# alebal123bal/BayesOpt_smart

Measured on AMD Instinct MI355X. Metric: candidate-points/sec (GP predict + HVI) at N_train=512, N_cand=1M, higher is better.
Workload: dtype f64; 1 GPU; C3: 2D/2-obj toy_function, N_train=512, N_cand=1,048,576 per GPU ('ij' integer grid), HVI (Sigma-UCB), q=3; n_train=512, n_cand_per_gpu=1048576, n_cand_total=1048576, n_objectives=2, dim=2, topq=3, parallelism=candidate-shard x1, step_launch=hip_graph, candidate_offset=0

## Files before the change

### bayesopt_smart_amd/csrc/bo_gridconv.hip

```cpp

#include "bo_predict_impl.h"

namespace {

using namespace bo;

constexpr int kListWaves = 4;
constexpr int kListChunk = 512;
#ifndef BO_ACC_RB
#define BO_ACC_RB 8
#endif
constexpr int kAccRB = BO_ACC_RB;
constexpr int kAccRows = 64 * kAccRB;
constexpr int kAccUnroll = 4;
constexpr int kClassLists = kConvClasses * kConvShards;
static_assert(kClassLists % 64 == 0 && kClassLists <= 2 * 64 * kConvAccWaves &&
              (kConvShards & (kConvShards - 1)) == 0 && kConvShards <= 16 && kConvShards <= kConvCountStride,
              "conv_acc_kernel's scan and lookup of the class lists");
#ifndef BO_CONV_PF
#define BO_CONV_PF 3
#endif
constexpr int kConvPF = BO_CONV_PF;
constexpr int kContractWaves = 8;
constexpr size_t kConvLdsBytes = 160 * 1024;
constexpr double kPairDrop = 0x1p-100;
constexpr double kTabFlush = 0x1p-128;

struct ListLds {
  int order, rc, nm;
  size_t bytes;
  __host__ __device__ ListLds(int n, int C)
      : order(C + 1), rc(order + n), nm(rc + 2 * n), bytes((size_t)(nm + kListWaves * kListChunk) * sizeof(int)) {}
};
struct AccLds {
  int ints, part;
  size_t bytes;
  __host__ __device__ explicit AccLds(int R)
      : ints(4 * R), part(kClassLists + 1),
        bytes((size_t)ints * sizeof(double) + (size_t)(part + kConvAccWaves + 1) / 2 * 2 * sizeof(int)) {}
};
struct ContractLds {
  int HB, tabH, hband, cn;
  size_t bytes;
  __host__ __device__ ContractLds(int C, int Cpad, int LT, int NP, int lists = 0)
      : HB(Cpad + LT / 2), tabH(2 * HB), hband(tabH + Cpad + C - 1), cn(hband + 1),
        bytes((size_t)cn * sizeof(double) + (size_t)NP * sizeof(int)) {
    if (bytes < (size_t)lists * sizeof(TopEntry)) bytes = (size_t)lists * sizeof(TopEntry);
  }
};

__device__ __forceinline__ void conv_list_done(const ConvArgs& a, int tau, int kept, int lane, int dyn) {
  if (kept == 0) {
    for (int o = 0; o < a.n_obj; ++o) {
      double* row = a.T + ((size_t)o * a.LT + tau) * a.ldr;
      for (int i = lane; i < a.ldr; i += 64) row[i] = 0.0;
    }
  }
  if (lane == 0) {
    a.pkept[tau] = kept;
    if (dyn && kept > 0) {
      const int e = 31 - __clz(kept);
      const int cls = 2 * e + (e > 0 ? (kept >> (e - 1)) & 1 : 0);
      const int sh = tau & (kConvShards - 1);
      const int slot = atomicAdd(a.ccount + cls * kConvCountStride + sh, 1);
      a.clist[(size_t)(cls * kConvShards + sh) * (a.LT / kConvShards) + slot] = tau;
    }
  }
}

__global__ __launch_bounds__(64 * kListWaves) void conv_list_kernel(const ConvArgs a, int tau_blocks, int dyn) {
  if (__builtin_amdgcn_readfirstlane(*a.flag) != 0) return;
  const int tid = threadIdx.x;
  if ((int)blockIdx.x >= tau_blocks) {
    const long long total = (long long)a.NP * a.ldr;
    const long long stride = (long long)(gridDim.x - tau_blocks) * (64 * kListWaves);
    for (int o = 0; o < a.n_obj; ++o) {
      const double nhl = a.nhl[o], pv = a.pv[o];
      double* tm = a.Tm + (size_t)o * a.NP * a.ldr;
      for (long long t = (long long)(blockIdx.x - tau_blocks) * (64 * kListWaves) + tid; t < total; t += stride) {
        const int s = (int)(t / a.ldr), i = (int)(t - (long long)s * a.ldr);
        double v = 0.0;
        if (s < a.n && i < a.nrows) {
          const int n = a.order[s];
          const double d = (double)(a.row_lo + i - a.rc[2 * n]);
          v = pv * a.alpha[(size_t)o * a.n_pad + n] * exp(nhl * (d * d));
        }
        tm[t] = v;
      }
    }
    return;
  }
  extern __shared__ __attribute__((aligned(16))) int si[];
  const ListLds L(a.n, a.C);
  int* cstart = si;
  int* order = si + L.order;
  int* rc = si + L.rc;
  for (int t = tid; t <= a.C; t += 64 * kListWaves) cstart[t] = a.cstart[t];
  for (int t = tid; t < a.n; t += 64 * kListWaves) order[t] = a.order[t];
  for (int t = tid; t < 2 * a.n; t += 64 * kListWaves) rc[t] = a.rc[t];
  __syncthreads();
  const int lane = tid & 63, wave = tid >> 6;
  int* nm = si + L.nm + wave * kListChunk;
  const int tau = blockIdx.x * kListWaves + wave;
  if (tau >= a.LT) return;
  int s0 = 0, s1 = 0;
  for (int c = lane; c < a.C; c += 64) {
    const int h = cstart[c + 1] - cstart[c];
    const int x0 = tau - c, x1 = x0 + 1;
    s0 += h * cstart[x0 < 0 ? 0 : x0 > a.C ? a.C : x0];
    s1 += h * cstart[x1 < 0 ? 0 : x1 > a.C ? a.C : x1];
  }
#pragma unroll
  for (int d = 32; d > 0; d >>= 1) {
    s0 += __shfl_xor(s0, d, 64);
    s1 += __shfl_xor(s1, d, 64);
  }
  const int h0 = (tau + 1) >> 1, h1 = (tau + 2) >> 1;
  const int p0 = __builtin_amdgcn_readfirstlane((s0 + cstart[h0 > a.C ? a.C : h0]) >> 1);
  const int total = __builtin_amdgcn_readfirstlane((s1 + cstart[h1 > a.C ? a.C : h1]) >> 1) - p0;
  if (lane == 0) a.pstart[tau] = p0;
  if (total == 0) {
    conv_list_done(a, tau, 0, lane, dyn);
    return;
  }
  const int R2 = 2 * a.R;
  const int per = (a.n + 63) / 64;
  const int n_lo = lane * per < a.n ? lane * per : a.n;
  const int n_hi = n_lo + per < a.n ? n_lo + per : a.n;
// ... 86 lines not shown
    const double* e = tb + s;
#pragma unroll
    for (int k = 0; k < kAccRB; ++k) ev[k] = e[it[k]];
  };
  auto term = [&](double wv, const double (&ev)[kAccRB]) {
#pragma unroll
    for (int k = 0; k < kAccRB; ++k) {
      const double t = __dmul_rn(wv, ev[k]);
      const double te = __builtin_fma(wv, ev[k], -t);
      const double s2 = __dadd_rn(hi[k], t);
      const double bb = __dsub_rn(s2, hi[k]);
      const double se = __dadd_rn(__dsub_rn(hi[k], __dsub_rn(s2, bb)), __dsub_rn(t, bb));
      hi[k] = s2;
      lo[k] = __dadd_rn(lo[k], __dadd_rn(se, te));
    }
  };
  int p = 0;
  for (; p + kAccUnroll <= cnt; p += kAccUnroll) {
    double wv[kAccUnroll];
    int sv[kAccUnroll];
#pragma unroll
    for (int u = 0; u < kAccUnroll; ++u) {
      wv[u] = w[p + u];
      sv[u] = sl[p + u];
    }
    double ev[2][kAccRB];
    gather(sv[0], ev[0]);
#pragma unroll
    for (int u = 0; u < kAccUnroll; ++u) {
      if (u + 1 < kAccUnroll) gather(sv[u + 1], ev[(u + 1) & 1]);
      term(wv[u], ev[u & 1]);
    }
  }
  for (; p < cnt; ++p) {
    double ev[kAccRB];
    gather(sl[p], ev);
    term(w[p], ev);
  }
#pragma unroll
  for (int k = 0; k < kAccRB; ++k) {
    const int i = ib + lane + 64 * k;
    if (FULL) Trow[i] = hi[k] + lo[k];
    else if (i < ldr) Trow[i] = i < nrows ? hi[k] + lo[k] : 0.0;
  }
}

__global__ __launch_bounds__(64 * kConvAccWaves) void conv_acc_kernel(
    const ConvArgs a, const double* __restrict__ pair_w, const int* __restrict__ pair_sl,
    const int* __restrict__ pstart, const int* __restrict__ pkept, const int* __restrict__ ccount,
    const int* __restrict__ clist, int* __restrict__ ticket, double* __restrict__ T, int nrb, int ngrp, int dyn) {
  if (__builtin_amdgcn_readfirstlane(*a.flag) != 0) return;
  extern __shared__ __attribute__((aligned(16))) double sd[];
  const int tid = threadIdx.x, lane = tid & 63, o = blockIdx.y;
  const double nhl = a.nhl[o];
  const int R2 = 2 * a.R;
  const AccLds L(a.R);
  double* tabE = sd;
  int* cst = (int*)(sd + L.ints);
  int* part = cst + L.part;
  for (int t = tid; t < 2 * R2; t += 64 * kConvAccWaves) {
    const int par = t >= R2 ? 1 : 0, h = t - par * R2;
    const double m = (double)(2 * h + par - (R2 - 2));
    tabE[t] = exp(0.5 * nhl * (m * m));
  }
  if (dyn) {
    int c[2], sum = 0;
#pragma unroll
    for (int u = 0; u < 2; ++u) {
      const int j = 2 * tid + u;
      c[u] = j < kClassLists ? ccount[(kConvClasses - 1 - j / kConvShards) * kConvCountStride + j % kConvShards] : 0;
      sum += c[u];
    }
    int incl = sum;
#pragma unroll
    for (int d = 1; d < 64; d <<= 1) {
      const int v = __shfl_up(incl, d, 64);
      if (lane >= d) incl += v;
    }
    if (lane == 63) part[tid >> 6] = incl;
    __syncthreads();
    int run = incl - sum;
    for (int w = 0; w < (tid >> 6); ++w) run += part[w];
#pragma unroll
    for (int u = 0; u < 2; ++u) {
      const int j = 2 * tid + u;
      if (j < kClassLists) cst[j] = run;
      run += c[u];
      if (j == kClassLists - 1) cst[kClassLists] = run;
    }
  }
  __syncthreads();
  const int n_items = (dyn ? cst[kClassLists] : a.LT) * nrb;
  const double* wo = pair_w + (size_t)o * a.n_pairs;
  const int g = blockIdx.x % ngrp;
  int* tk = ticket + (o * kConvTicketGroups + g) * kConvTicketStride;
  for (int k = (blockIdx.x / ngrp) * kConvAccWaves + (tid >> 6);;) {
    const int t = k * ngrp + g;
    if (t >= n_items) break;
    int nx = 0;
    if (dyn && lane == 0) nx = atomicAdd(tk, 1);
    const int oi = t / nrb, rb = t - oi * nrb;
    int tau = oi;
    if (dyn) {
      constexpr int per = kClassLists / 64;
      const unsigned long long b1 = __ballot(cst[per * lane + per] > oi);
      const int l1 = __builtin_ctzll(b1);
      const unsigned long long b2 = __ballot(cst[per * l1 + (lane < per ? lane : per - 1) + 1] > oi);
      const int j = per * l1 + __builtin_ctzll(b2);
      const int cls = kConvClasses - 1 - j / kConvShards;
      const int* list = clist + (size_t)(cls * kConvShards + j % kConvShards) * (a.LT / kConvShards);
      tau = __builtin_amdgcn_readfirstlane(list[oi - cst[j]]);
    }
    const int p0 = __builtin_amdgcn_readfirstlane(pstart[tau]);
    const int cnt = __builtin_amdgcn_readfirstlane(pkept[tau]);
    if (!dyn && cnt == 0) break;
    const int ib = rb * kAccRows;
    double* Trow = T + ((size_t)o * a.LT + tau) * a.ldr;
// ... 13 lines not shown
#pragma unroll
  for (int s = 0; s < 4; ++s) v[s] = p[(size_t)s * ldr];
#endif
}

template <int NB, class BGen>
__device__ __forceinline__ void conv_gemm(const double* __restrict__ X, int ldr, int nkb, int g, d4 (&acc)[NB],
                                          BGen&& bgen) {
  double ring[kConvPF][4];
#pragma unroll
  for (int p = 0; p < kConvPF; ++p) conv_load_a(X, ldr, p < nkb ? p : nkb - 1, g, ring[p]);
  for (int kb0 = 0; kb0 < nkb; kb0 += kConvPF) {
#pragma unroll
    for (int p = 0; p < kConvPF; ++p) {
      const int kb = kb0 + p;
      if (kb < nkb) {
        double av[4];
#pragma unroll
        for (int s = 0; s < 4; ++s) av[s] = ring[p][s];
        const int nx = kb + kConvPF;
        conv_load_a(X, ldr, nx < nkb ? nx : nkb - 1, g, ring[p]);
        double bv[4][NB];
        bgen(kb, bv);
#pragma unroll
        for (int s = 0; s < 4; ++s)
#pragma unroll
          for (int nb = 0; nb < NB; ++nb) acc[nb] = mfma64(av[s], bv[s][nb], acc[nb]);
      }
    }
  }
}

template <int NB>
__global__ __launch_bounds__(64 * kContractWaves) void conv_contract_kernel(const ConvArgs a) {
  if (__builtin_amdgcn_readfirstlane(*a.flag) != 0) return;
  extern __shared__ __attribute__((aligned(16))) double sd[];
  const ContractLds L(a.C, a.Cpad, a.LT, a.NP);
  double* tabB = sd;
  double* tabH = sd + L.tabH;
  int* hband = (int*)(sd + L.hband);
  int* cn = (int*)(sd + L.cn);
  constexpr int TW = 16 * NB;
  const int tid = threadIdx.x, lane = tid & 63, wave = tid >> 6;
  const int nt = blockDim.x, W = nt >> 6;
  const int g = lane >> 4, jl = lane & 15;
  const int cb_n = a.Cpad / TW;
  const long long n_wt = (long long)(a.ldr / 16) * cb_n;
  const long long gi_lo = a.cand_offset, gi_hi = a.cand_offset + a.n_cand;
#ifndef BO_ABL_CT_NOOUT
  const bool outs = true;
#else
  const bool outs = a.ld_out < 0;
#endif
  for (int t = tid; t < a.NP; t += nt) cn[t] = t < a.n ? a.rc[2 * a.order[t] + 1] : 0;

  double lv = -__builtin_inf();
  long long li = -1;
  double tab_nhl = __builtin_nan("");
  for (long long base = (long long)blockIdx.x * W; base < n_wt; base += (long long)gridDim.x * W) {
    const long long wt = base + wave;
    const bool active = wt < n_wt;
    const long long wtc = active ? wt : n_wt - 1;
    const int i0 = (int)(wtc / cb_n) * 16, j0 = (int)(wtc % cb_n) * TW;
    double acq[NB][4];
    for (int o = 0; o < a.n_obj; ++o) {
      const double nhl = a.nhl[o];
      if (!(nhl == tab_nhl)) {
        __syncthreads();
        int mq = 0;
        int mm = 0;
#ifndef BO_ABL_CT_NOTAB
        for (int t = tid; t < 2 * L.HB; t += nt) {
          const int par = t >= L.HB ? 1 : 0, h = t - par * L.HB;
          const int mi = 2 * h + par - (a.LT - 1);
          const double m = (double)mi;
          const double v = exp(0.5 * nhl * (m * m));
          const bool flush = v < kTabFlush;
          tabB[t] = flush ? 0.0 : v;
          if (!flush) mq = max(mq, abs(mi));
        }
        for (int t = tid; t < a.Cpad + a.C - 1; t += nt) {
          const int mi = t - (a.C - 1);
          const double m = (double)mi;
          const double v = exp(nhl * (m * m));
          const bool flush = v < kTabFlush;
          tabH[t] = flush ? 0.0 : v;
          if (!flush) mm = max(mm, abs(mi));
        }
#else
        mm = min((int)sqrt(128.0 * 0.6931471805599453 / -nhl), a.C - 1);
        mq = min((int)sqrt(256.0 * 0.6931471805599453 / -nhl), a.LT - 1);
#endif
        if (tid < 2) hband[tid] = 0;
        __syncthreads();
#pragma unroll
        for (int d = 32; d > 0; d >>= 1) {
          mq = max(mq, __shfl_xor(mq, d, 64));
          mm = max(mm, __shfl_xor(mm, d, 64));
        }
        if (lane == 0) {
          atomicMax(hband, mq);
          atomicMax(hband + 1, mm);
        }
        __syncthreads();
        tab_nhl = nhl;
      }
      int kq_lo = 0, kq_hi = a.LT / 16;
      if (!a.full) {
        const int hq = hband[0];
        const int t_hi = 2 * (j0 + TW - 1) + hq < a.LT - 1 ? 2 * (j0 + TW - 1) + hq : a.LT - 1;
        const int t_lo = 2 * j0 - hq > 0 ? (2 * j0 - hq < t_hi ? 2 * j0 - hq : t_hi) : 0;
        kq_lo = __builtin_amdgcn_readfirstlane(t_lo >> 4);
        kq_hi = __builtin_amdgcn_readfirstlane((t_hi >> 4) + 1);
      }
      d4 aq[NB], am[NB];
#pragma unroll
      for (int nb = 0; nb < NB; ++nb) {
        aq[nb] = (d4){0.0, 0.0, 0.0, 0.0};
        am[nb] = (d4){0.0, 0.0, 0.0, 0.0};
      }
      const double* Tq = a.T + ((size_t)o * a.LT + 16 * kq_lo) * a.ldr + i0 + jl;
      int km_lo = 0, km_hi = a.NP / 16;
      if (!a.full) {
        const int hm = hband[1];
        const int c_hi = j0 + TW + hm < a.C ? j0 + TW + hm : a.C;
        const int c_lo = j0 - hm > 0 ? (j0 - hm < a.C ? j0 - hm : a.C) : 0;
        km_lo = __builtin_amdgcn_readfirstlane(a.cstart[c_lo] >> 4);
        km_hi = __builtin_amdgcn_readfirstlane((a.cstart[c_hi] + 15) >> 4);
      }
      const double* Tm = a.Tm + ((size_t)o * a.NP + 16 * km_lo) * a.ldr + i0 + jl;
      const double* pe0 = tabB + (a.LT / 2 - 1 - 8 * kq_lo - 2 * g) + j0 + jl;
#ifdef BO_ABL_CT_BCONST
      const double bconst = pe0[0];
#endif
      conv_gemm<NB>(Tq, a.ldr, kq_hi - kq_lo, g, aq, [&](int kb, double (&bv)[4][NB]) {
#ifdef BO_ABL_CT_BCONST
#pragma unroll
        for (int s = 0; s < 4; ++s)
#pragma unroll
          for (int nb = 0; nb < NB; ++nb) bv[s][nb] = bconst;
#else
        const double* pe = pe0 - 8 * kb;
        const double* po = pe + L.HB;
#pragma unroll
        for (int nb = 0; nb < NB; ++nb) {
          bv[0][nb] = po[16 * nb];
          bv[1][nb] = pe[16 * nb];
          bv[2][nb] = po[16 * nb - 1];
          bv[3][nb] = pe[16 * nb - 1];
        }
#endif
      });
      const int* cn0 = cn + 16 * km_lo + 4 * g;
      if (km_hi > km_lo) conv_gemm<NB>(Tm, a.ldr, km_hi - km_lo, g, am, [&](int kb, double (&bv)[4][NB]) {
#ifdef BO_ABL_CT_BCONST
#pragma unroll
        for (int s = 0; s < 4; ++s)
#pragma unroll
          for (int nb = 0; nb < NB; ++nb) bv[s][nb] = bconst;
#else
        const int* c4 = cn0 + 16 * kb;
        const double* ph = tabH + j0 + jl + (a.C - 1);
#pragma unroll
        for (int s = 0; s < 4; ++s) {
          const double* p = ph - c4[s];
#pragma unroll
          for (int nb = 0; nb < NB; ++nb) bv[s][nb] = p[16 * nb];
        }
#endif
      });
      if constexpr (NB == 1) {
        mfma_fence<false>(aq[0], am[0]);
      } else {
#pragma unroll
        for (int nb = 0; nb < NB; nb += 2) {
          mfma_fence<false>(aq[nb], aq[nb + 1]);
          mfma_fence<false>(am[nb], am[nb + 1]);
        }
      }
      const double pv = a.pv[o], pm = a.pm[o];
#pragma unroll
      for (int nb = 0; nb < NB; ++nb) {
#pragma unroll
        for (int r = 0; r < 4; ++r) {
          const double mu = pm + am[nb][r];
          const double var = fmax(pv - aq[nb][r], a.min_var);
          const double smu = (mu - pm) * a.inv_rsq_pv[o];
          const double svar = var * a.inv_pv[o];
          const double u = smu + a.beta[o] * sqrt(fabs(svar));
          acq[nb][r] = (o == 0) ? u : acq[nb][r] + u;
          const int row = a.row_lo + i0 + g + 4 * r, c = j0 + 16 * nb + jl;
          const long long gi = (long long)row * a.C + c;
          if (outs && active && i0 + g + 4 * r < a.nrows && c < a.C && gi >= gi_lo && gi < gi_hi) {
            const long long off = (long long)o * a.ld_out + (gi - gi_lo);
            if (a.mu) bo_out_store(a.mu + off, mu);
            if (a.var) bo_out_store(a.var + off, var);
            if (a.std_mu) bo_out_store(a.std_mu + off, smu);
            if (a.std_var) bo_out_store(a.std_var + off, svar);
            if (a.ucb) bo_out_store(a.ucb + off, u);
          }
        }
      }
    }
    long long gis[NB][4];
#pragma unroll
    for (int nb = 0; nb < NB; ++nb) {
#pragma unroll
      for (int r = 0; r < 4; ++r) {
        const int row = a.row_lo + i0 + g + 4 * r, c = j0 + 16 * nb + jl;
        const long long gi = (long long)row * a.C + c;
        const bool ok = active && i0 + g + 4 * r < a.nrows && c < a.C && gi >= gi_lo && gi < gi_hi;
        gis[nb][r] = ok ? gi : -1;
        if (outs && ok && a.acq) bo_out_store(a.acq + (gi - gi_lo), acq[nb][r]);
      }
    }
#ifndef BO_ABL_CT_NOSEL
    const bool select = a.topq > 0;
#else
    const bool select = a.topq > 0 && a.n_lists < 0;
#endif
    if (select) {
      const int q = a.topq;
      const unsigned long long kq = bo_readlane_u(bo_order_key(lv, li), q - 1);
      const long long iq = bo_readlane_i(li, q - 1);
      bool beats = false;
#pragma unroll
      for (int nb = 0; nb < NB; ++nb)
#pragma unroll
        for (int r = 0; r < 4; ++r)
          beats = beats || bo_key_before(bo_order_key(acq[nb][r], gis[nb][r]), gis[nb][r], kq, iq);
      if (__ballot(beats) != 0ull) {
        unsigned int taken = 0;
        double nv = -__builtin_inf();
        long long ni = -1;
        int filled = 0;
        while (filled < q) {
          unsigned long long bk = 0ull;
          long long bi = -1;
          int bs = -1;
#pragma unroll
          for (int nb = 0; nb < NB; ++nb) {
#pragma unroll
            for (int r = 0; r < 4; ++r) {
              const int s = 4 * nb + r;
              const unsigned long long k = ((taken >> s) & 1u) ? 0ull : bo_order_key(acq[nb][r], gis[nb][r]);
              if (bo_key_before(k, gis[nb][r], bk, bi)) { bk = k; bi = gis[nb][r]; bs = s; }
            }
          }
          {
            const unsigned long long k = (lane < q && !((taken >> 16) & 1u)) ? bo_order_key(lv, li) : 0ull;
            if (bo_key_before(k, li, bk, bi)) { bk = k; bi = li; bs = 16; }
          }
          unsigned long long wk = bk;
          long long wi = bi;
#pragma unroll
          for (int m = 32; m > 0; m >>= 1) {
            const unsigned long long ok = __shfl_xor(wk, m, 64);
            const long long oi = __shfl_xor(wi, m, 64);
            if (bo_key_before(ok, oi, wk, wi)) { wk = ok; wi = oi; }
          }
          if (wk == 0ull) break;
          const bool win = bk == wk && bi == wi;
          bool excluded = false;
          if (win) {
            taken |= 1u << bs;
            if (bs != 16) {
              const long long row = wi / a.C, c = wi - row * a.C;
              double co[BO_MAX_DIM] = {(double)(a.lo0 + row), (double)(a.lo1 + c), 0.0, 0.0, 0.0, 0.0, 0.0, 0.0};
              excluded = bo_hash_contains(a.hkeys, a.hidx, a.hmask, a.excl_pts, 2, co, 2);
            }
          }
          if (__ballot(excluded) != 0ull) continue;
          if (lane == filled) { nv = bo_key_value(wk); ni = wi; }
          ++filled;
        }
        lv = nv;
        li = ni;
      }
    }
  }
  if (a.topq > 0) {
    const int q = a.topq;
    TopEntry* ml = (TopEntry*)sd;
    __syncthreads();
    if (lane < q) {
      ml[wave * q + lane].v = lv;
      ml[wave * q + lane].i = li;
    }
    __syncthreads();
    if (wave == 0) {
      int head = 0;
      double nv = -__builtin_inf();
      long long ni = -1;
      for (int r = 0; r < q; ++r) {
        const bool has = lane < W && head < q;
        const double hv = has ? ml[lane * q + head].v : -__builtin_inf();
        const long long hi = has ? ml[lane * q + head].i : -1;
        const unsigned long long bk = bo_order_key(hv, hi);
        unsigned long long wk = bk;
        long long wi = hi;
#pragma unroll
        for (int m = 32; m > 0; m >>= 1) {
          const unsigned long long ok = __shfl_xor(wk, m, 64);
          const long long oi = __shfl_xor(wi, m, 64);
          if (bo_key_before(ok, oi, wk, wi)) { wk = ok; wi = oi; }
        }
        if (wk == 0ull) break;
        const bool win = bk == wk && hi == wi;
        if (win) ++head;
        const double wv = __shfl(hv, __builtin_ctzll(__ballot(win)), 64);
        if (lane == r) { nv = wv; ni = wi; }
      }
      if (lane < q) {
        TopEntry* dst = a.partial + (size_t)blockIdx.x * q;
        dst[lane].v = nv;
        dst[lane].i = ni;
      }
    }
    if (blockIdx.x == 0) {
      const long long e0 = (long long)gridDim.x * q, e1 = (long long)a.n_lists * q;
      for (long long e = e0 + tid; e < e1; e += nt) {
        a.partial[e].v = -__builtin_inf();
        a.partial[e].i = -1;
      }
    }
  }
}

}

namespace bo {

bool conv_lds_admits(int n, int R, int C, int Cpad, int LT, int NP) {
  const size_t bound = ((size_t)4 * R + 2048) * sizeof(double) + ((size_t)(C + 1) + 3 * (size_t)n + 2048) * sizeof(int);
  assert(ConvSetupLds(n, C, 256).bytes <= bound && ListLds(n, C).bytes <= bound && AccLds(R).bytes <= bound);
  return bound <= kConvLdsBytes && ContractLds(C, Cpad, LT, NP).bytes <= kConvLdsBytes;
}

template <class K>
static hipError_t conv_lds_attr(K k, size_t lds) {
  if (lds <= 64 * 1024) return hipSuccess;
  return hipFuncSetAttribute((const void*)k, hipFuncAttributeMaxDynamicSharedMemorySize, (int)lds);
}

ConvSched conv_acc_schedule(int R, int LT, int ldr, int n_obj, int cus) {
  ConvSched sc;
  sc.nrb = (ldr + kAccRows - 1) / kAccRows;
  const long long items = (long long)LT * sc.nrb;
  const size_t tab = (size_t)4 * R * sizeof(double);
  const int per_cu = (int)(kConvLdsBytes / tab < 4 ? kConvLdsBytes / tab : 4);
  long long wgs = (long long)(cus > 0 ? cus : 256) * per_cu / n_obj;
  if (wgs > (items + kConvAccWaves - 1) / kConvAccWaves) wgs = (items + kConvAccWaves - 1) / kConvAccWaves;
  if (wgs < 1) wgs = 1;
  sc.wgs = (int)wgs;
  sc.ngrp = (int)(wgs < kConvTicketGroups ? wgs : kConvTicketGroups);
  sc.dyn = (items <= wgs * kConvAccWaves && wgs % sc.ngrp == 0) ? 0 : 1;
  return sc;
}

hipError_t launch_gridconv(const ConvArgs& ca, const ConvPlan& cp, const ConvSched& sc, hipStream_t st) {
  const size_t l1 = ListLds(ca.n, ca.C).bytes, la = AccLds(ca.R).bytes;
  const size_t l2 = ContractLds(ca.C, ca.Cpad, ca.LT, ca.NP, cp.waves * ca.topq).bytes;
  if (l1 > kConvLdsBytes || la > kConvLdsBytes) return hipErrorInvalidValue;
  if (cp.waves < 1 || cp.waves > kContractWaves || cp.grid > ca.n_lists) return hipErrorInvalidValue;
  auto* contract = cp.nb == 4 ? conv_contract_kernel<4> : cp.nb == 2 ? conv_contract_kernel<2> : conv_contract_kernel<1>;
  hipError_t e;
  if ((e = conv_lds_attr(conv_list_kernel, l1)) != hipSuccess) return e;
  if ((e = conv_lds_attr(conv_acc_kernel, la)) != hipSuccess) return e;
  if ((e = conv_lds_attr(contract, l2)) != hipSuccess) return e;
  const int tau_blocks = (ca.LT + kListWaves - 1) / kListWaves;
  const long long tm_elems = (long long)ca.NP * ca.ldr;
  const int tm_blocks = (int)((tm_elems + 1023) / 1024 < 512 ? (tm_elems + 1023) / 1024 : 512);
  hipLaunchKernelGGL(conv_list_kernel, dim3(tau_blocks + tm_blocks), dim3(64 * kListWaves), l1, st, ca, tau_blocks,
                     sc.dyn);
  if ((e = hipGetLastError()) != hipSuccess) return e;
  hipLaunchKernelGGL(conv_acc_kernel, dim3((unsigned)sc.wgs, ca.n_obj), dim3(64 * kConvAccWaves), la, st, ca,
                     (const double*)ca.pair_w, (const int*)ca.pair_sl, (const int*)ca.pstart, (const int*)ca.pkept,
                     (const int*)ca.ccount, (const int*)ca.clist, ca.ticket, ca.T, sc.nrb, sc.ngrp, sc.dyn);
  if ((e = hipGetLastError()) != hipSuccess) return e;
  hipLaunchKernelGGL(contract, dim3(cp.grid), dim3(64 * cp.waves), l2, st, ca);
  return hipGetLastError();
}

}
```

### bayesopt_smart_amd/csrc/bo_predict.hip

```cpp

#include "bo_predict_impl.h"

#include <vector>

namespace {

__device__ __forceinline__ double kstar_at(const FusedArgs& a, int o, int f, long long j, bool valid) {
  return (valid && f < a.n_train) ? a.kstar[((long long)o * a.ks_rows + f) * a.n_cand + j] : 0.0;
}

template <int NS, bool SELECT>
__device__ __forceinline__ void contract_epair(__amdgpu_buffer_rsrc_t wr, int voff, int base,
                                               int& pos, int ep, const double (&B)[NS],
                                               d2 (&wa)[kPF], d2 (&wb)[kPF], d4& acc0, d4& acc1,
                                               double (&sel0)[4], double (&sel1)[4]) {
  constexpr int NCH = NS / 8;
#pragma unroll
  for (int c = 0; c < NCH; ++c) {
#pragma unroll
    for (int pp = 0; pp < 4; ++pp) {
      const int p = 4 * c + pp;
      const d2 ca = wa[pp];
      const d2 cb = wb[pp];
      const int so = base + ((pos + kPF) << 11);
// ... 400 lines not shown
  return cus;
}

constexpr double kConvMargin = 1.15;
constexpr int kConvMaxN = 4096;

void plan_gridconv(const bo_predict_desc* d, Plan* pl, bool kmem, int cus) {
  if (kmem || !pl->cm || d->cand_kind != BO_CAND_GRID || d->dim != 2 || d->n_cand <= 0) return;
  if (d->mode & (BO_PREDICT_DENSE | BO_PREDICT_NO_SEPARABLE | BO_PREDICT_FP32 | BO_PREDICT_NO_GRID_CONV)) return;
  const char* env = getenv("BO_GRID_CONV");
  if (env && env[0] == '0' && env[1] == 0) return;
  const long long R = d->grid_shape[0], C = d->grid_shape[1], n = d->n_train;
  if (R < 1 || C < 1 || R > (1 << 15) || C > (1 << 15) || n > kConvMaxN) return;
  if (d->cand_offset < 0 || d->cand_offset + d->n_cand > R * C) return;
  bo::ConvPlan cp = {};
  cp.row_lo = (int)(d->cand_offset / C);
  cp.nrows = (int)((d->cand_offset + d->n_cand - 1) / C) - cp.row_lo + 1;
  cp.ldr = (cp.nrows + 15) / 16 * 16;
  cp.Cpad = (int)((C + 63) / 64 * 64);
  cp.LT = (int)((2 * C - 1 + 15) / 16 * 16);
  cp.NP = (int)((n + 15) / 16 * 16);
  if (!bo::conv_lds_admits((int)n, (int)R, (int)C, cp.Cpad, cp.LT, cp.NP)) return;
  const long long wave_tiles = (long long)(cp.ldr / 16) * (cp.Cpad / 64);
  if (!(d->mode & (BO_PREDICT_GRID_CONV | BO_PREDICT_GRID_CONV_FULL))) {
    const double nch = pl->n_pad / 32;
    const double F = (double)d->n_obj * 1024.0 * nch * (nch + 1);
    const double old_rounds = (double)(((d->n_cand + 63) / 64 + 255) / 256);
    const double old_us = 25.0 + old_rounds * 64.0 * (F / 273.0e3 + 0.038);
    const double pairs_per_tau = 0.5 * (double)n * (double)(n + 1) / (double)(2 * C - 1);
    const double pair_us = 2.2 * pairs_per_tau * (double)((cp.ldr + 1023) / 1024) *
                           (double)((d->n_obj * (2 * C - 1) + 4095) / 4096);
    const double tile_rounds = (double)((wave_tiles + 1023) / 1024);
    const double contract_us = tile_rounds * 2048.0 * (double)(cp.LT + cp.NP) * (double)d->n_obj / 48.8e3;
    const double conv_us = 60.0 + pair_us + contract_us;
    if (!(kConvMargin * conv_us < old_us)) return;
  }
  cp.planned = true;
  const long long tiles64 = wave_tiles;
  cp.nb = tiles64 >= 8LL * cus ? 4 : 2 * tiles64 >= 8LL * cus ? 2 : 1;
  const char* tile = getenv("BO_CONV_TILE");
  if (tile && (tile[0] == '1' || tile[0] == '2' || tile[0] == '4') && tile[1] == 0) cp.nb = tile[0] - '0';
  const long long tiles = tiles64 * (4 / cp.nb);
  cp.waves = tiles >= 8LL * cus ? 8 : 4;
  long long wgs = (tiles + cp.waves - 1) / cp.waves;
#ifdef BO_ABL_CT_W4
  cp.waves = 4;
  wgs = (tiles + 3) / 4;
  if (wgs > 2LL * cus) wgs = 2LL * cus;
#else
  if (wgs > cus) wgs = cus;
#endif
  if (wgs > (long long)pl->grid * pl->waves) wgs = (long long)pl->grid * pl->waves;
  cp.grid = (int)wgs;
  cp.ws = bo::conv_layout(n, d->n_obj, C, cp.LT, cp.NP, cp.ldr, align256(pl->total));
  pl->total = cp.ws.end;
  pl->conv = cp;
}

int make_plan(const bo_predict_desc* d, Plan* pl, bool query_device, bool kmem = false) {
  if (!d || d->n_obj < 1 || d->n_obj > BO_MAX_OBJ || d->dim < 1 || d->dim > BO_MAX_DIM)
    return BO_ERR_ARG;
  if (d->n_train < 1 || d->n_cand < 0 || d->topq < 0 || d->topq > BO_MAX_TOPQ) return BO_ERR_ARG;
  if (d->cand_kind < 0 || d->cand_kind > BO_CAND_SOBOL) return BO_ERR_ARG;
  if (d->mode & ~(BO_PREDICT_DENSE | BO_PREDICT_NO_SEPARABLE | BO_PREDICT_FP32 | BO_PREDICT_F32_FLOOR |
                  BO_PREDICT_NO_GRID_CONV | BO_PREDICT_GRID_CONV | BO_PREDICT_GRID_CONV_FULL))
    return BO_ERR_ARG;
  if (d->excl_points && d->n_excl < 0) return BO_ERR_ARG;
  const long long n = d->n_train;
  if (n > (1 << 14)) return BO_ERR_UNSUPPORTED;
  memset(pl, 0, sizeof(*pl));
  pl->dim_pad = pad_dim(d->dim);
  pl->n_excl = (int)(d->excl_points ? d->n_excl : n);
  pl->n_panels = 1;
  if ((d->mode & BO_PREDICT_FP32) && !kmem) {
    const int n_pad = (int)((n + 63) / 64 * 64);
    const size_t lds = ((size_t)n_pad * pl->dim_pad + (size_t)d->n_obj * n_pad) * sizeof(float);
    if (lds <= kLdsBytes) {
      pl->fp32 = true;
      pl->n_pad = n_pad;
      pl->ns = 16;
      pl->lds = lds;
    }
  }
  if (!pl->fp32 && !kmem) {
    const int n_pad = pad_rows(n);
    const size_t base = (size_t)n_pad * pl->dim_pad + (size_t)d->n_obj * n_pad;
    pl->cm = true;
    pl->n_pad = n_pad;
    pl->ns = n_pad / 4;
    const size_t plain = base + bo::kExpTab;
    size_t lds = plain;
    if (d->cand_kind == BO_CAND_GRID && !(d->mode & BO_PREDICT_NO_SEPARABLE)) {
      const long long S = d->grid_shape[d->dim - 1];
      const size_t tbl = (size_t)d->n_obj * (2 * S - 1);
      const size_t rw_c = (size_t)n_pad * (d->n_obj + 1) + (size_t)(S + 63) / 64;
      const size_t lds_c = base + tbl + (size_t)kWaves * rw_c;
      const size_t lds_1 = base + tbl + (size_t)kWaves * n_pad * 2;
      if (S % 16 == 0 && S <= 32768 && d->cand_offset % 16 == 0 && lds_1 <= kLdsDoubles) {
        pl->sep = true;
        pl->rw_cache = lds_c <= kLdsDoubles;
        pl->rw_stride = (int)(pl->rw_cache ? rw_c : (size_t)n_pad * 2);
        pl->off_tbl = (int)base;
        pl->off_rw = (int)(base + tbl);
        lds = pl->rw_cache ? lds_c : lds_1;
        if (lds < plain) lds = plain;
      }
    }
// ... 184 lines not shown
  fa.off_tbl = pl.off_tbl;
  fa.off_rw = pl.off_rw;
  fa.rw_cache = pl.rw_cache ? 1 : 0;
  fa.rw_stride = pl.rw_stride;
  fa.off_exp = pl.off_exp;
  fa.conv_flag = pl.conv.planned ? (int*)(ws + pl.off_status + 32) : nullptr;
  return BO_OK;
}

static void fill_conv_args(const bo_predict_desc* d, const Plan& pl, char* ws, const FusedArgs& fa, bo::ConvArgs& ca) {
  const bo::ConvPlan& cp = pl.conv;
  const bo::ConvLayout& L = cp.ws;
  memset(&ca, 0, sizeof(ca));
  ca.n_obj = d->n_obj;
  ca.n = (int)d->n_train;
  ca.n_pad = pl.n_pad;
  ca.R = (int)d->grid_shape[0];
  ca.C = (int)d->grid_shape[1];
  ca.lo0 = d->grid_lo[0];
  ca.lo1 = d->grid_lo[1];
  ca.cand_offset = d->cand_offset;
  ca.n_cand = d->n_cand;
  ca.ld_out = fa.ld_out;
  ca.row_lo = cp.row_lo;
  ca.nrows = cp.nrows;
  ca.ldr = cp.ldr;
  ca.LT = cp.LT;
  ca.NP = cp.NP;
  ca.Cpad = cp.Cpad;
  ca.flag = (int*)fa.conv_flag;
  ca.x = d->x_train;
  ca.kinv = d->kinv;
  ca.ld_k = d->ld_k;
  ca.alpha = fa.alpha;
  memcpy(ca.pm, fa.pm, sizeof(ca.pm));
  memcpy(ca.pv, fa.pv, sizeof(ca.pv));
  memcpy(ca.nhl, fa.nhl, sizeof(ca.nhl));
  memcpy(ca.beta, fa.beta, sizeof(ca.beta));
  memcpy(ca.inv_rsq_pv, fa.inv_rsq_pv, sizeof(ca.inv_rsq_pv));
  memcpy(ca.inv_pv, fa.inv_pv, sizeof(ca.inv_pv));
  ca.min_var = fa.min_var;
  ca.cstart = (int*)(ws + L.cstart);
  ca.order = (int*)(ws + L.order);
  ca.rc = (int*)(ws + L.rc);
  ca.pstart = (int*)(ws + L.pstart);
  ca.pkept = (int*)(ws + L.pkept);
  ca.clist = (int*)(ws + L.clist);
  ca.ticket = (int*)(ws + L.ticket);
  ca.ccount = (int*)(ws + L.ccount);
  ca.Tm = (double*)(ws + L.Tm);
  ca.T = (double*)(ws + L.T);
  ca.pair_sl = (int*)(ws + L.pair_sl);
  ca.pair_w = (double*)(ws + L.pair_w);
  ca.n_pairs = (int)(d->n_train * (d->n_train + 1) / 2);
  ca.full = (d->mode & BO_PREDICT_GRID_CONV_FULL) ? 1 : 0;
  ca.mu = fa.mu;
  ca.var = fa.var;
  ca.std_mu = fa.std_mu;
  ca.std_var = fa.std_var;
  ca.ucb = fa.ucb;
  ca.acq = fa.acq;
  ca.topq = d->topq;
  ca.partial = fa.partial;
  ca.n_lists = pl.grid * pl.waves;
  ca.excl_pts = fa.excl ? fa.excl : fa.xpad;
  ca.hkeys = fa.hkeys;
  ca.hidx = fa.hidx;
  ca.hmask = fa.hmask;
}

static size_t fill_prep_args(const bo_predict_desc* d, const Plan& pl, char* ws, bool kmem, const FusedArgs& fa,
                             PrepArgs& pa) {
  memset(&pa, 0, sizeof(pa));
  pa.pack_mode = pl.fp32 ? 2 : (pl.cm ? 0 : 1);
  pa.wpack = ws;
  pa.kinv = d->kinv;
  pa.ld_k = d->ld_k;
  pa.upper = fa.upper;
  pa.n = (int)d->n_train;
  pa.n_pad = pl.n_pad;
  pa.ns = pl.ns;
  pa.n_obj = d->n_obj;
  const long long total = pl.fp32 ? c32_blocks(pl.n_pad / 64) * 1024 * d->n_obj
                        : pl.cm ? cm_blocks(pl.n_pad / 32, fa.upper) * 512 * d->n_obj
                                : (long long)d->n_obj * pl.n_pad * pl.n_pad / 2;
  pa.pack_blocks = (int)((total + 255) / 256 < 2048 ? (total + 255) / 256 : 2048);
  pa.alpha_blocks = (int)(((long long)d->n_obj * pl.n_pad + 3) / 4);
  pa.alpha = (double*)fa.alpha;
  pa.y = d->y_train;
  pa.ld_y = d->ld_y;
  for (int o = 0; o < d->n_obj; ++o) pa.pm[o] = d->prior_mean[o];
  pa.rows = kmem ? 0 : 1;
  pa.xpad = (double*)fa.xpad;
  pa.xc = (double*)fa.xc;
  pa.x = d->x_train;
  pa.dim = d->dim;
  pa.DIM = pl.dim_pad;
  pa.sep_flag = (int*)fa.sep_flag;
  pa.sep_lo = fa.sep_lo;
  pa.sep_S = fa.sep_S;
  pa.excl = (double*)(ws + pl.off_excl);
  pa.excl_in = d->excl_points;
  pa.n_excl = (kmem || !d->excl_points) ? 0 : pl.n_excl;
  pa.hkeys = (unsigned long long*)fa.hkeys;
  pa.hidx = (int*)fa.hidx;
  pa.hslots = pl.hash_slots;
  pa.n_hash = (kmem || d->topq == 0) ? 0 : pl.n_excl;
  pa.hash_lds = pa.n_hash > 0 && pl.hash_slots <= 2048 ? 1 : 0;
  return pa.hash_lds ? (size_t)pl.hash_slots * 12 : 0;
}

static int predict_impl(const bo_predict_desc* d, const double* kstar, long long ks_rows,
                        void* workspace, size_t ws_bytes, void* stream) {
  const bool kmem = kstar != nullptr;
  Plan pl;
  int st = make_plan(d, &pl, true, kmem);
  if (st != BO_OK) return st;
// ... 153 lines not shown
```

### bayesopt_smart_amd/csrc/bo_predict_impl.h

```cpp
#pragma once

#include "bo_common.h"

#include <assert.h>
#include <math.h>
#include <stdlib.h>
#include <string.h>

#include <type_traits>

namespace bo {

constexpr int kWaves = 4;
constexpr int kTile = 16 * kWaves;
constexpr int kPanelSteps = 128;
constexpr int kPF = 4;
constexpr int kCMaxEp = 16;
constexpr int kC32MaxEp = 16;
using ::kExpTab;

struct FusedArgs {
  int n_obj, dim, n_train, n_pad;
  int n_panels;
  int n_excl;
// ... 6 lines not shown
  const double* excl;
  const d2* wpack;
  unsigned int wpack_bytes;
  int w_pairs;
  const double* alpha;
  double pm[BO_MAX_OBJ], pv[BO_MAX_OBJ], nhl[BO_MAX_OBJ], beta[BO_MAX_OBJ];
  double inv_rsq_pv[BO_MAX_OBJ], inv_pv[BO_MAX_OBJ];
  double min_var;
  int idx32;
  double *mu, *var, *std_mu, *std_var, *ucb, *acq;
  TopEntry* partial;
  const double* kstar;
  long long ks_rows;
  int upper;
  const int* sep_flag;
  int sep_S;
  long long sep_lo;
  int off_tbl, off_rw;
  int rw_cache;
  int rw_stride;
  int off_exp;
  SobolArgs sob;
  const unsigned long long* hkeys;
  const int* hidx;
  unsigned int hmask;
  const int* conv_flag;
};

struct ConvArgs {
  int n_obj, n, n_pad;
  int R, C;
  long long lo0, lo1;
  long long cand_offset, n_cand, ld_out;
  int row_lo, nrows, ldr;
  int LT;
  int NP;
  int Cpad;
  int* flag;
  const double* x;
  const double* kinv;
  long long ld_k;
  const double* alpha;
  double pm[BO_MAX_OBJ], pv[BO_MAX_OBJ], nhl[BO_MAX_OBJ], beta[BO_MAX_OBJ];
  double inv_rsq_pv[BO_MAX_OBJ], inv_pv[BO_MAX_OBJ];
  double min_var;
  int* cstart;
  int* order;
  int* rc;
  int* pstart;
  int* pkept;
  int* ccount;
  int* clist;
  int* ticket;
  int n_pairs;
  int* pair_sl;
  double* pair_w;
  double* T;
  double* Tm;
  double *mu, *var, *std_mu, *std_var, *ucb, *acq;
  int topq;
  int full;
  TopEntry* partial;
  int n_lists;
  const double* excl_pts;
  const unsigned long long* hkeys;
  const int* hidx;
  unsigned int hmask;
};

constexpr int kConvTicketGroups = 32;
constexpr int kConvTicketStride = 32;
constexpr int kConvClasses = 64;
#ifndef BO_CONV_SHARDS
#define BO_CONV_SHARDS 8
#endif
constexpr int kConvShards = BO_CONV_SHARDS;
constexpr int kConvCountStride = 32;
constexpr int kConvAccWaves = 4;

struct ConvSched {
  int nrb;
  int wgs, ngrp;
  int dyn;
};

struct ConvSetupLds {
  int col, part;
  size_t bytes;
  __host__ __device__ ConvSetupLds(int n, int C, int threads)
      : col(C + 1), part(col + n), bytes((size_t)(part + threads / 64) * sizeof(int)) {}
};

template <int THREADS>
__device__ __forceinline__ void conv_scan(int* v, int len, int* part, int* out) {
  const int tid = threadIdx.x, lane = tid & 63, wave = tid >> 6;
  const int seg = (len + THREADS - 1) / THREADS;
  const int c_lo = tid * seg < len ? tid * seg : len, c_hi = c_lo + seg < len ? c_lo + seg : len;
  int sum = 0;
  for (int c = c_lo; c < c_hi; ++c) sum += v[c];
  int incl = sum;
#pragma unroll
  for (int d = 1; d < 64; d <<= 1) {
    const int t = __shfl_up(incl, d, 64);
    if (lane >= d) incl += t;
  }
  if (lane == 63) part[wave] = incl;
  __syncthreads();
  int run = incl - sum;
  for (int w = 0; w < wave; ++w) run += part[w];
  for (int c = c_lo; c < c_hi; ++c) {
    const int t = v[c];
    v[c] = run;
    if (out) out[c] = run;
    run += t;
  }
  __syncthreads();
}

template <int THREADS>
__device__ __forceinline__ void conv_setup_block(const ConvArgs& a, const ConvSched& sc, int* lds) {
  const ConvSetupLds L(a.n, a.C, THREADS);
  int* cnt = lds;
  int* col = lds + L.col;
  int* part = lds + L.part;
  const int tid = threadIdx.x, lane = tid & 63;
  for (int c = tid; c <= a.C; c += THREADS) cnt[c] = 0;
  for (int t = tid; t < a.n_obj * sc.ngrp; t += THREADS) {
    const int g = t % sc.ngrp;
    a.ticket[(t / sc.ngrp * kConvTicketGroups + g) * kConvTicketStride] =
        (sc.wgs - g + sc.ngrp - 1) / sc.ngrp * kConvAccWaves;
  }
  for (int t = tid; t < kConvClasses * kConvShards; t += THREADS)
    a.ccount[t / kConvShards * kConvCountStride + t % kConvShards] = 0;
  __syncthreads();
  for (int n = tid; n < a.n; n += THREADS) {
    const int r = (int)fmin(fmax(a.x[2 * (long long)n] - (double)a.lo0, 0.0), (double)(a.R - 1));
    const int c = (int)fmin(fmax(a.x[2 * (long long)n + 1] - (double)a.lo1, 0.0), (double)(a.C - 1));
    a.rc[2 * n] = r;
    a.rc[2 * n + 1] = c;
    col[n] = c;
    atomicAdd(cnt + c, 1);
  }
  __syncthreads();
  conv_scan<THREADS>(cnt, a.C + 1, part, a.cstart);
  if (tid >= 64) return;
  const int bits = a.C > 1 ? 32 - __clz(a.C - 1) : 0;
  for (int n0 = 0; n0 < a.n; n0 += 64) {
    const int n = n0 + lane;
    const bool valid = n < a.n;
    const int c = valid ? col[n] : 0;
    unsigned long long m = __ballot(valid);
    for (int b = 0; b < bits; ++b) {
      const bool bit = (c >> b) & 1;
      const unsigned long long bal = __ballot(valid && bit);
      m &= bit ? bal : ~bal;
    }
    const unsigned long long below = m & ((1ull << lane) - 1ull);
    const int base = valid ? cnt[c] : 0;
    __builtin_amdgcn_fence(__ATOMIC_RELEASE, "wavefront");
    __builtin_amdgcn_wave_barrier();
    __builtin_amdgcn_fence(__ATOMIC_ACQUIRE, "wavefront");
    if (valid) {
      a.order[base + __popcll(below)] = n;
      if (below == 0ull) cnt[c] = base + __popcll(m);
    }
    __builtin_amdgcn_fence(__ATOMIC_RELEASE, "wavefront");
    __builtin_amdgcn_wave_barrier();
    __builtin_amdgcn_fence(__ATOMIC_ACQUIRE, "wavefront");
  }
}

struct ConvLayout {
  size_t cstart, order, rc, pstart, pkept, clist, ticket, ccount, Tm, T, pair_sl, pair_w, end;
};

inline ConvLayout conv_layout(long long n, int n_obj, long long C, long long LT, long long NP, long long ldr,
                              size_t base) {
  size_t at = base;
  auto take = [&at](long long count, size_t elem, size_t align) {
    const size_t off = (at + align - 1) / align * align;
    at = off + (size_t)count * elem;
    return off;
  };
  const long long pairs = n * (n + 1) / 2;
  ConvLayout L;
  L.cstart = take(C + 1, sizeof(int), 256);
  L.order = take(n, sizeof(int), sizeof(int));
  L.rc = take(2 * n, sizeof(int), sizeof(int));
  L.pstart = take(LT, sizeof(int), sizeof(int));
  L.pkept = take(LT, sizeof(int), sizeof(int));
  L.clist = take(kConvClasses * LT, sizeof(int), sizeof(int));
  L.ticket = take(BO_MAX_OBJ * kConvTicketGroups * kConvTicketStride, sizeof(int), 128);
  L.ccount = take(kConvClasses * kConvCountStride, sizeof(int), 128);
  L.Tm = take(n_obj * NP * ldr, sizeof(double), 256);
  L.T = take(n_obj * LT * ldr, sizeof(double), 256);
  L.pair_sl = take(pairs, sizeof(int), 256);
  L.pair_w = take(n_obj * pairs, sizeof(double), 256);
  L.end = take(0, 1, 256) + (L.ticket % 256 == 0 ? 256 : 0);
  return L;
}

bool conv_lds_admits(int n, int R, int C, int Cpad, int LT, int NP);
ConvSched conv_acc_schedule(int R, int LT, int ldr, int n_obj, int cus);

struct ConvPlan {
  bool planned;
  int nb;
  int waves;
  int grid;
  int row_lo, nrows, ldr, LT, NP, Cpad;
  ConvLayout ws;
};

hipError_t launch_gridconv(const ConvArgs& ca, const ConvPlan& cp, const ConvSched& sc, hipStream_t st);

struct Plan {
  int n_pad, ns, n_panels, dim_pad, n_excl;
  bool multi;
  size_t off_alpha, off_xpad, off_xc, off_excl, off_hash, off_partial, off_status, total;
  unsigned int hash_slots;
  bool cm;
  bool sep;
  bool grows;
  int off_tbl, off_rw;
  bool rw_cache;
  int rw_stride;
  bool fp32;
  bool small;
  int off_exp;
  int grid, waves;
  long long n_tiles;
  size_t lds;
  ConvPlan conv;
};

hipError_t launch_cm_d2(const Plan& pl, const FusedArgs& fa, hipStream_t st);
hipError_t launch_cm_d4(const Plan& pl, const FusedArgs& fa, hipStream_t st);
hipError_t launch_cm_d6(const Plan& pl, const FusedArgs& fa, hipStream_t st);
hipError_t launch_cm_d8(const Plan& pl, const FusedArgs& fa, hipStream_t st);
hipError_t launch_c32_d2(const Plan& pl, const FusedArgs& fa, hipStream_t st);
hipError_t launch_c32_d4(const Plan& pl, const FusedArgs& fa, hipStream_t st);
hipError_t launch_c32_d6(const Plan& pl, const FusedArgs& fa, hipStream_t st);
hipError_t launch_c32_d8(const Plan& pl, const FusedArgs& fa, hipStream_t st);
hipError_t launch_cms_d2(const Plan& pl, const FusedArgs& fa, hipStream_t st);
hipError_t launch_cms_d4(const Plan& pl, const FusedArgs& fa, hipStream_t st);
hipError_t launch_cms_d6(const Plan& pl, const FusedArgs& fa, hipStream_t st);
hipError_t launch_cms_d8(const Plan& pl, const FusedArgs& fa, hipStream_t st);

}

namespace {
// ... 973 lines not shown
```

Baseline: 5.433 billion candidate-points/sec.

## Precompute exp tables once per objective and prefilter training-point exclusion by tile

The exp lookup tables and band widths used by the accumulate and contract kernels are now built once per distinct length-scale by extra blocks in the list kernel and stored in workspace. The later kernels copy them into LDS instead of recomputing the exponentials in every workgroup. The contract kernel also packs row and column into the cn array, so the training points lying inside a tile can be marked taken up front. This replaces the per-winner hash lookup when the exclusion set is the training set. The cost is extra global memory traffic, an extra workspace region, and more coupling between the kernels.

```diff
diff --git a/bayesopt_smart_amd/csrc/bo_gridconv.hip b/bayesopt_smart_amd/csrc/bo_gridconv.hip
--- a/bayesopt_smart_amd/csrc/bo_gridconv.hip
+++ b/bayesopt_smart_amd/csrc/bo_gridconv.hip
@@ -68,12 +68,64 @@
   }
 }
 
-__global__ __launch_bounds__(64 * kListWaves) void conv_list_kernel(const ConvArgs a, int tau_blocks, int dyn) {
+__device__ __forceinline__ void conv_tables(const ConvArgs& a, int t0, int nthr, int lane) {
+  const int R2 = 2 * a.R;
+  const ContractLds L(a.C, a.Cpad, a.LT, a.NP);
+  for (int o = 0; o < a.n_obj; ++o) {
+    if (a.tix[o] != o) continue;
+    const double nhl = a.nhl[o];
+    double* tabE = a.tabE + (size_t)o * 2 * R2;
+    for (int t = t0; t < 2 * R2; t += nthr) {
+      const int par = t >= R2 ? 1 : 0, h = t - par * R2;
+      const double m = (double)(2 * h + par - (R2 - 2));
+      tabE[t] = exp(0.5 * nhl * (m * m));
+    }
+    double* tabB = a.ctab + (size_t)o * conv_ctab_doubles(a.C, a.Cpad, a.LT);
+    double* tabH = tabB + L.tabH;
+    int mq = 0;
+    int mm = 0;
+    for (int t = t0; t < 2 * L.HB; t += nthr) {
+      const int par = t >= L.HB ? 1 : 0, h = t - par * L.HB;
+      const int mi = 2 * h + par - (a.LT - 1);
+      const double m = (double)mi;
+      const double v = exp(0.5 * nhl * (m * m));
+      const bool flush = v < kTabFlush;
+      tabB[t] = flush ? 0.0 : v;
+      if (!flush) mq = max(mq, abs(mi));
+    }
+    for (int t = t0; t < a.Cpad + a.C - 1; t += nthr) {
+      const int mi = t - (a.C - 1);
+      const double m = (double)mi;
+      const double v = exp(nhl * (m * m));
+      const bool flush = v < kTabFlush;
+      tabH[t] = flush ? 0.0 : v;
+      if (!flush) mm = max(mm, abs(mi));
+    }
+#pragma unroll
+    for (int d = 32; d > 0; d >>= 1) {
+      mq = max(mq, __shfl_xor(mq, d, 64));
+      mm = max(mm, __shfl_xor(mm, d, 64));
+    }
+    if (lane == 0) {
+      int* hband = (int*)(tabB + L.hband);
+      atomicMax(hband, mq);
+      atomicMax(hband + 1, mm);
+    }
+  }
+}
+
+__global__ __launch_bounds__(64 * kListWaves) void conv_list_kernel(const ConvArgs a, int tau_blocks, int tm_blocks,
+                                                                    int dyn) {
   if (__builtin_amdgcn_readfirstlane(*a.flag) != 0) return;
   const int tid = threadIdx.x;
+  if ((int)blockIdx.x >= tau_blocks + tm_blocks) {
+    conv_tables(a, (blockIdx.x - tau_blocks - tm_blocks) * (64 * kListWaves) + tid,
+                (gridDim.x - tau_blocks - tm_blocks) * (64 * kListWaves), tid & 63);
+    return;
+  }
   if ((int)blockIdx.x >= tau_blocks) {
     const long long total = (long long)a.NP * a.ldr;
-    const long long stride = (long long)(gridDim.x - tau_blocks) * (64 * kListWaves);
+    const long long stride = (long long)tm_blocks * (64 * kListWaves);
     for (int o = 0; o < a.n_obj; ++o) {
       const double nhl = a.nhl[o], pv = a.pv[o];
       double* tm = a.Tm + (size_t)o * a.NP * a.ldr;
@@ -266,17 +318,13 @@
   if (__builtin_amdgcn_readfirstlane(*a.flag) != 0) return;
   extern __shared__ __attribute__((aligned(16))) double sd[];
   const int tid = threadIdx.x, lane = tid & 63, o = blockIdx.y;
-  const double nhl = a.nhl[o];
   const int R2 = 2 * a.R;
   const AccLds L(a.R);
   double* tabE = sd;
   int* cst = (int*)(sd + L.ints);
   int* part = cst + L.part;
-  for (int t = tid; t < 2 * R2; t += 64 * kConvAccWaves) {
-    const int par = t >= R2 ? 1 : 0, h = t - par * R2;
-    const double m = (double)(2 * h + par - (R2 - 2));
-    tabE[t] = exp(0.5 * nhl * (m * m));
-  }
+  const double2* te = (const double2*)(a.tabE + (size_t)a.tix[o] * 2 * R2);
+  for (int t = tid; t < R2; t += 64 * kConvAccWaves) ((double2*)tabE)[t] = te[t];
   if (dyn) {
     int c[2], sum = 0;
 #pragma unroll
@@ -396,11 +444,14 @@
 #else
   const bool outs = a.ld_out < 0;
 #endif
-  for (int t = tid; t < a.NP; t += nt) cn[t] = t < a.n ? a.rc[2 * a.order[t] + 1] : 0;
+  for (int t = tid; t < a.NP; t += nt) {
+    const int n = t < a.n ? a.order[t] : -1;
+    cn[t] = n >= 0 ? a.rc[2 * n + 1] | (a.rc[2 * n] << 16) : 0;
+  }
 
   double lv = -__builtin_inf();
   long long li = -1;
-  double tab_nhl = __builtin_nan("");
+  int tab_ix = -1;
   for (long long base = (long long)blockIdx.x * W; base < n_wt; base += (long long)gridDim.x * W) {
     const long long wt = base + wave;
     const bool active = wt < n_wt;
@@ -408,46 +459,14 @@
     const int i0 = (int)(wtc / cb_n) * 16, j0 = (int)(wtc % cb_n) * TW;
     double acq[NB][4];
     for (int o = 0; o < a.n_obj; ++o) {
-      const double nhl = a.nhl[o];
-      if (!(nhl == tab_nhl)) {
+      const int tx = a.tix[o];
+      if (tx != tab_ix) {
         __syncthreads();
-        int mq = 0;
-        int mm = 0;
-#ifndef BO_ABL_CT_NOTAB
-        for (int t = tid; t < 2 * L.HB; t += nt) {
-          const int par = t >= L.HB ? 1 : 0, h = t - par * L.HB;
-          const int mi = 2 * h + par - (a.LT - 1);
-          const double m = (double)mi;
-          const double v = exp(0.5 * nhl * (m * m));
-          const bool flush = v < kTabFlush;
-          tabB[t] = flush ? 0.0 : v;
-          if (!flush) mq = max(mq, abs(mi));
-        }
-        for (int t = tid; t < a.Cpad + a.C - 1; t += nt) {
-          const int mi = t - (a.C - 1);
-          const double m = (double)mi;
-          const double v = exp(nhl * (m * m));
-          const bool flush = v < kTabFlush;
-          tabH[t] = flush ? 0.0 : v;
-          if (!flush) mm = max(mm, abs(mi));
-        }
-#else
-        mm = min((int)sqrt(128.0 * 0.6931471805599453 / -nhl), a.C - 1);
-        mq = min((int)sqrt(256.0 * 0.6931471805599453 / -nhl), a.LT - 1);
-#endif
-        if (tid < 2) hband[tid] = 0;
+        const double* src = a.ctab + (size_t)tx * conv_ctab_doubles(a.C, a.Cpad, a.LT);
+        for (int t = tid; t < L.cn / 2; t += nt) ((double2*)sd)[t] = ((const double2*)src)[t];
+        if ((L.cn & 1) && tid == 0) sd[L.cn - 1] = src[L.cn - 1];
         __syncthreads();
-#pragma unroll
-        for (int d = 32; d > 0; d >>= 1) {
-          mq = max(mq, __shfl_xor(mq, d, 64));
-          mm = max(mm, __shfl_xor(mm, d, 64));
-        }
-        if (lane == 0) {
-          atomicMax(hband, mq);
-          atomicMax(hband + 1, mm);
-        }
-        __syncthreads();
-        tab_nhl = nhl;
+        tab_ix = tx;
       }
       int kq_lo = 0, kq_hi = a.LT / 16;
       if (!a.full) {
@@ -507,7 +526,7 @@
         const double* ph = tabH + j0 + jl + (a.C - 1);
 #pragma unroll
         for (int s = 0; s < 4; ++s) {
-          const double* p = ph - c4[s];
+          const double* p = ph - (c4[s] & 0xffff);
 #pragma unroll
           for (int nb = 0; nb < NB; ++nb) bv[s][nb] = p[16 * nb];
         }
@@ -575,6 +594,20 @@
           beats = beats || bo_key_before(bo_order_key(acq[nb][r], gis[nb][r]), gis[nb][r], kq, iq);
       if (__ballot(beats) != 0ull) {
         unsigned int taken = 0;
+        if (a.excl_train) {
+          const int s_hi = __builtin_amdgcn_readfirstlane(a.cstart[j0 + TW < a.C ? j0 + TW : a.C]);
+          for (int s0 = __builtin_amdgcn_readfirstlane(a.cstart[j0 < a.C ? j0 : a.C]); s0 < s_hi; s0 += 64) {
+            const int e = s0 + lane < s_hi ? cn[s0 + lane] : 0;
+            const int dr = (e >> 16) - (a.row_lo + i0), dc = (e & 0xffff) - j0;
+            unsigned long long hits = __ballot(s0 + lane < s_hi && dr >= 0 && dr < 16);
+            while (hits != 0ull) {
+              const int src = __builtin_ctzll(hits);
+              hits &= hits - 1ull;
+              const int hr = __builtin_amdgcn_readlane(dr, src), hc = __builtin_amdgcn_readlane(dc, src);
+              if (lane == 16 * (hr & 3) + (hc & 15)) taken |= 1u << (4 * (hc >> 4) + (hr >> 2));
+            }
+          }
+        }
         double nv = -__builtin_inf();
         long long ni = -1;
         int filled = 0;
@@ -608,7 +641,7 @@
           bool excluded = false;
           if (win) {
             taken |= 1u << bs;
-            if (bs != 16) {
+            if (bs != 16 && !a.excl_train) {
               const long long row = wi / a.C, c = wi - row * a.C;
               double co[BO_MAX_DIM] = {(double)(a.lo0 + row), (double)(a.lo1 + c), 0.0, 0.0, 0.0, 0.0, 0.0, 0.0};
               excluded = bo_hash_contains(a.hkeys, a.hidx, a.hmask, a.excl_pts, 2, co, 2);
@@ -678,6 +711,7 @@
 bool conv_lds_admits(int n, int R, int C, int Cpad, int LT, int NP) {
   const size_t bound = ((size_t)4 * R + 2048) * sizeof(double) + ((size_t)(C + 1) + 3 * (size_t)n + 2048) * sizeof(int);
   assert(ConvSetupLds(n, C, 256).bytes <= bound && ListLds(n, C).bytes <= bound && AccLds(R).bytes <= bound);
+  assert(ContractLds(C, Cpad, LT, NP).hband == conv_ctab_band(C, Cpad, LT));
   return bound <= kConvLdsBytes && ContractLds(C, Cpad, LT, NP).bytes <= kConvLdsBytes;
 }
 
@@ -715,8 +749,10 @@
   const int tau_blocks = (ca.LT + kListWaves - 1) / kListWaves;
   const long long tm_elems = (long long)ca.NP * ca.ldr;
   const int tm_blocks = (int)((tm_elems + 1023) / 1024 < 512 ? (tm_elems + 1023) / 1024 : 512);
-  hipLaunchKernelGGL(conv_list_kernel, dim3(tau_blocks + tm_blocks), dim3(64 * kListWaves), l1, st, ca, tau_blocks,
-                     sc.dyn);
+  const long long tab_elems = 4LL * ca.R > 2LL * ca.Cpad + ca.LT ? 4LL * ca.R : 2LL * ca.Cpad + ca.LT;
+  const int tab_blocks = (int)((tab_elems + 255) / 256 < 64 ? (tab_elems + 255) / 256 : 64);
+  hipLaunchKernelGGL(conv_list_kernel, dim3(tau_blocks + tm_blocks + tab_blocks), dim3(64 * kListWaves), l1, st, ca,
+                     tau_blocks, tm_blocks, sc.dyn);
   if ((e = hipGetLastError()) != hipSuccess) return e;
   hipLaunchKernelGGL(conv_acc_kernel, dim3((unsigned)sc.wgs, ca.n_obj), dim3(64 * kConvAccWaves), la, st, ca,
                      (const double*)ca.pair_w, (const int*)ca.pair_sl, (const int*)ca.pstart, (const int*)ca.pkept,
diff --git a/bayesopt_smart_amd/csrc/bo_predict.hip b/bayesopt_smart_amd/csrc/bo_predict.hip
--- a/bayesopt_smart_amd/csrc/bo_predict.hip
+++ b/bayesopt_smart_amd/csrc/bo_predict.hip
@@ -476,7 +476,7 @@
 #endif
   if (wgs > (long long)pl->grid * pl->waves) wgs = (long long)pl->grid * pl->waves;
   cp.grid = (int)wgs;
-  cp.ws = bo::conv_layout(n, d->n_obj, C, cp.LT, cp.NP, cp.ldr, align256(pl->total));
+  cp.ws = bo::conv_layout(n, d->n_obj, R, C, cp.Cpad, cp.LT, cp.NP, cp.ldr, align256(pl->total));
   pl->total = cp.ws.end;
   pl->conv = cp;
 }
@@ -767,6 +767,13 @@
   ca.T = (double*)(ws + L.T);
   ca.pair_sl = (int*)(ws + L.pair_sl);
   ca.pair_w = (double*)(ws + L.pair_w);
+  ca.tabE = (double*)(ws + L.tabE);
+  ca.ctab = (double*)(ws + L.ctab);
+  for (int o = 0; o < d->n_obj; ++o) {
+    int t = 0;
+    while (memcmp(&ca.nhl[t], &ca.nhl[o], sizeof(double)) != 0) ++t;
+    ca.tix[o] = t;
+  }
   ca.n_pairs = (int)(d->n_train * (d->n_train + 1) / 2);
   ca.full = (d->mode & BO_PREDICT_GRID_CONV_FULL) ? 1 : 0;
   ca.mu = fa.mu;
@@ -778,6 +785,7 @@
   ca.topq = d->topq;
   ca.partial = fa.partial;
   ca.n_lists = pl.grid * pl.waves;
+  ca.excl_train = fa.excl ? 0 : 1;
   ca.excl_pts = fa.excl ? fa.excl : fa.xpad;
   ca.hkeys = fa.hkeys;
   ca.hidx = fa.hidx;
diff --git a/bayesopt_smart_amd/csrc/bo_predict_impl.h b/bayesopt_smart_amd/csrc/bo_predict_impl.h
--- a/bayesopt_smart_amd/csrc/bo_predict_impl.h
+++ b/bayesopt_smart_amd/csrc/bo_predict_impl.h
@@ -82,6 +82,9 @@
   int* ccount;
   int* clist;
   int* ticket;
+  int tix[BO_MAX_OBJ];
+  double* tabE;
+  double* ctab;
   int n_pairs;
   int* pair_sl;
   double* pair_w;
@@ -92,6 +95,7 @@
   int full;
   TopEntry* partial;
   int n_lists;
+  int excl_train;
   const double* excl_pts;
   const unsigned long long* hkeys;
   const int* hidx;
@@ -107,6 +111,13 @@
 constexpr int kConvShards = BO_CONV_SHARDS;
 constexpr int kConvCountStride = 32;
 constexpr int kConvAccWaves = 4;
+
+__host__ __device__ inline long long conv_ctab_band(long long C, long long Cpad, long long LT) {
+  return 2 * (Cpad + LT / 2) + Cpad + C - 1;
+}
+__host__ __device__ inline long long conv_ctab_doubles(long long C, long long Cpad, long long LT) {
+  return (conv_ctab_band(C, Cpad, LT) + 1 + 1) / 2 * 2;
+}
 
 struct ConvSched {
   int nrb;
@@ -162,6 +173,9 @@
   }
   for (int t = tid; t < kConvClasses * kConvShards; t += THREADS)
     a.ccount[t / kConvShards * kConvCountStride + t % kConvShards] = 0;
+  if (tid < a.n_obj) {
+    a.ctab[tid * conv_ctab_doubles(a.C, a.Cpad, a.LT) + conv_ctab_band(a.C, a.Cpad, a.LT)] = 0.0;
+  }
   __syncthreads();
   for (int n = tid; n < a.n; n += THREADS) {
     const int r = (int)fmin(fmax(a.x[2 * (long long)n] - (double)a.lo0, 0.0), (double)(a.R - 1));
@@ -201,11 +215,11 @@
 }
 
 struct ConvLayout {
-  size_t cstart, order, rc, pstart, pkept, clist, ticket, ccount, Tm, T, pair_sl, pair_w, end;
+  size_t cstart, order, rc, pstart, pkept, clist, ticket, ccount, Tm, T, pair_sl, pair_w, tabE, ctab, end;
 };
 
-inline ConvLayout conv_layout(long long n, int n_obj, long long C, long long LT, long long NP, long long ldr,
-                              size_t base) {
+inline ConvLayout conv_layout(long long n, int n_obj, long long R, long long C, long long Cpad, long long LT,
+                              long long NP, long long ldr, size_t base) {
   size_t at = base;
   auto take = [&at](long long count, size_t elem, size_t align) {
     const size_t off = (at + align - 1) / align * align;
@@ -226,7 +240,10 @@
   L.T = take(n_obj * LT * ldr, sizeof(double), 256);
   L.pair_sl = take(pairs, sizeof(int), 256);
   L.pair_w = take(n_obj * pairs, sizeof(double), 256);
-  L.end = take(0, 1, 256) + (L.ticket % 256 == 0 ? 256 : 0);
+  at = take(0, 1, 256) + (L.ticket % 256 == 0 ? 256 : 0);
+  L.tabE = take(n_obj * 4 * R, sizeof(double), 256);
+  L.ctab = take(n_obj * conv_ctab_doubles(C, Cpad, LT), sizeof(double), 256);
+  L.end = take(0, 1, 256);
   return L;
 }
 
```

Result: faster. 5.597 billion candidate-points/sec, median of 6 (+3.0%).
